# hanmekim/SceneLib2

Hardware: AMD Instinct MI355X
Metric: batched MonoSLAM frames/sec (320x240, 100 feat) (higher is better)
Workload: dtype f64

## Files before the change

scenelib2_amd/csrc/sl2_ekf_update.hip:

```cpp
#include "sl2_common.hpp"
#include "sl2_chol_diag.hpp"

namespace sl2 {

typedef double v4d __attribute__((ext_vector_type(4)));

__device__ __forceinline__ v4d mfma_f64(double a, double b, v4d c) {
  return __builtin_amdgcn_mfma_f64_16x16x4f64(a, b, c, 0, 0, 0);
}

#ifdef SL2_TESTING
#define SL2_EKF_TEST_SECTION 1
#include "sl2_ekf_update_testing.inc"
#undef SL2_EKF_TEST_SECTION
#endif

constexpr int kASBatch = 4;

template <int NQ, int BATCH>
__global__ void __launch_bounds__(1024) k_build_AS(const double* __restrict__ P, const double* __restrict__ f_Hx,
                                                  const double* __restrict__ f_Hy, const double* __restrict__ f_nu,
                                                  const double* __restrict__ f_R, const int* __restrict__ succ_idx,
                                                  const int* __restrict__ m_count, double* __restrict__ At,
                                                  double* __restrict__ St, const int* __restrict__ f_hcol,
                                                  const int* __restrict__ pos_err_any, int N, int ld, int mld) {
  extern __shared__ double sAt[];
  const int b = blockIdx.x;
  const int cnt = m_count[b];
  if (cnt == 0) return;
  const int m = 2 * cnt, mp = (m + 31) / 32 * 32;
  const int t = threadIdx.x;
  double* Ab = At + (size_t)b * mld * ld;
  double* Sb = St + (size_t)b * mld * mld;
  const double* Pb = P + (size_t)b * ld * ld;
  const int* sidx = succ_idx + (size_t)b * N;
  const int* hcol = (pos_err_any[b] != 0) ? f_hcol + (size_t)b * N : nullptr;
  double pc[NQ][7];
#pragma unroll
  for (int q = 0; q < NQ; ++q) {
    const int i = t + q * (int)blockDim.x;
#pragma unroll
    for (int c = 0; c < 7; ++c) pc[q][c] = (i >= ld) ? 0.0 : ((i < 13) ? Pb[(size_t)i * ld + c] : Pb[(size_t)c * ld + i]);
  }
  double hx[7], hy[3], Rn = 0.0;
  int posa = 0;
  if (t < m) {
    const int fa = sidx[t >> 1];
    const size_t fia = (size_t)b * N + fa;
    posa = hcol ? hcol[fa] : 13 + 3 * fa;
#pragma unroll
    for (int c = 0; c < 7; ++c) hx[c] = (hcol && (unsigned)(c - posa) < 3u) ? 0.0 : f_Hx[fia * 14 + (t & 1) * 7 + c];
#pragma unroll
    for (int c = 0; c < 3; ++c) hy[c] = f_Hy[fia * 6 + (t & 1) * 3 + c];
    Rn = f_R[fia];
  }
  const int nbatch = (cnt + BATCH - 1) / BATCH, per = (nbatch + (int)gridDim.y - 1) / (int)gridDim.y;
  const int jbeg = (int)blockIdx.y * per * BATCH;
  const int jend = (jbeg + per * BATCH < cnt) ? jbeg + per * BATCH : cnt;
  for (int j0 = jbeg; j0 < jend; j0 += BATCH) {
    const int nb = (jend - j0 < BATCH) ? jend - j0 : BATCH;
#pragma unroll
    for (int jj = 0; jj < BATCH; ++jj) {
      if (jj < nb) {
        const int f = sidx[j0 + jj];
        const size_t fi = (size_t)b * N + f;
        const int pos = hcol ? hcol[f] : 13 + 3 * f;
#pragma unroll
        for (int q = 0; q < NQ; ++q) {
          const int i = t + q * (int)blockDim.x;
          if (i < ld) {
            double py[3];
#pragma unroll
            for (int c = 0; c < 3; ++c)
              py[c] = Pb[(size_t)(pos + c) * ld + i];
#pragma unroll
            for (int r = 0; r < 2; ++r) {
              double acc = 0.0;
#pragma unroll
              for (int c = 0; c < 7; ++c) acc += pc[q][c] * ((hcol && (unsigned)(c - pos) < 3u) ? 0.0 : f_Hx[fi * 14 + r * 7 + c]);
#pragma unroll
              for (int c = 0; c < 3; ++c) acc += py[c] * f_Hy[fi * 6 + r * 3 + c];
              if (i == ld - 1) acc = f_nu[fi * 2 + r];
              Ab[(size_t)(2 * (j0 + jj) + r) * ld + i] = acc;
              sAt[(2 * jj + r) * ld + i] = acc;
            }
          }
        }
      }
    }
    __syncthreads();
    if (t < mp) {
#pragma unroll
      for (int kk = 0; kk < 2 * BATCH; ++kk) {
        const int k = 2 * j0 + kk;
        if (kk < 2 * nb && (t | 31) >= k) {
          double v = 0.0;
          if (t < m) {
            const double* arow = sAt + kk * ld;
            double acc = 0.0;
#pragma unroll
            for (int c = 0; c < 7; ++c) acc += hx[c] * arow[c];
#pragma unroll
            for (int c = 0; c < 3; ++c) acc += hy[c] * arow[posa + c];
            if (t == k) acc += Rn;
            v = acc;
          }
          Sb[(size_t)k * mld + t] = v;
        }
      }
    }
    __syncthreads();
  }
  if (blockIdx.y != 0) return;
  for (int k = m; k < mp; ++k) {
#pragma unroll
    for (int q = 0; q < NQ; ++q) {
      const int i = t + q * (int)blockDim.x;
      if (i < ld) Ab[(size_t)k * ld + i] = 0.0;
    }
    if (t < mp && (t | 31) >= k) Sb[(size_t)k * mld + t] = (t == k) ? 1.0 : 0.0;
  }
}

constexpr int kAheadEntry = 24;
constexpr int kAheadLdsMax = 40960;

template <int BATCH>
struct AheadRows { double v[BATCH][3]; };

__device__ __forceinline__ int ahead_pos(const double* en) { return *(const int*)(en + 23); }

__device__ __forceinline__ double ahead_lane(double v, int l) {
  return __hiloint2double(__builtin_amdgcn_readlane(__double2hiint(v), l), __builtin_amdgcn_readlane(__double2loint(v), l));
}

typedef __attribute__((address_space(1))) double ahead_gdouble;
__device__ __forceinline__ ahead_gdouble* ahead_at(const double* row, int t) {
  unsigned long long a = (unsigned long long)row;
  asm("" : "+s"(a));
  return (ahead_gdouble*)(a + (unsigned)t * (unsigned)sizeof(double));
}

template <int BATCH, bool FULL>
__device__ __forceinline__ void ahead_load(AheadRows<BATCH>& w, const double* __restrict__ Pb, const double* tab, int j0, int nb,
                                           int ld, int t) {
#pragma unroll
  for (int jj = 0; jj < BATCH; ++jj) {
    if (FULL || jj < nb) {
      const int pos = __builtin_amdgcn_readfirstlane(ahead_pos(tab + (j0 + jj) * kAheadEntry));
#pragma unroll
      for (int c = 0; c < 3; ++c) w.v[jj][c] = *ahead_at(Pb + (size_t)(pos + c) * ld, t);
    }
  }
}

template <int BATCH, bool FULL, bool REFILL>
__device__ __forceinline__ void ahead_rows(AheadRows<BATCH>& w, const double (&pc)[7], const double* tab, const double* __restrict__ Pb,
                                           double* __restrict__ Ab, double* sAt, int j0, int nb, int ld, int t) {
#pragma unroll
  for (int jj = 0; jj < BATCH; ++jj) {
    if (FULL || jj < nb) {
      double en = 0.0;
      if ((t & 63) < kAheadEntry) en = tab[(j0 + jj) * kAheadEntry + (t & 63)];
#pragma unroll
      for (int r = 0; r < 2; ++r) {
        double acc = 0.0;
#pragma unroll
        for (int c = 0; c < 7; ++c) acc += pc[c] * ahead_lane(en, r * 7 + c);
#pragma unroll
        for (int c = 0; c < 3; ++c) acc += w.v[jj][c] * ahead_lane(en, 14 + r * 3 + c);
        if (t == ld - 1) acc = ahead_lane(en, 20 + r);
        *ahead_at(Ab + (size_t)(2 * (j0 + jj) + r) * ld, t) = acc;
        sAt[(2 * jj + r) * ld + t] = acc;
      }
      if (REFILL && jj < BATCH - 1) {
        const int pos = __builtin_amdgcn_readfirstlane(ahead_pos(tab + (j0 + BATCH + jj) * kAheadEntry));
#pragma unroll
        for (int c = 0; c < 3; ++c) w.v[jj][c] = *ahead_at(Pb + (size_t)(pos + c) * ld, t);
      }
    }
  }
}

template <int BATCH>
__device__ __forceinline__ void ahead_refill_last(AheadRows<BATCH>& w, const double* tab, const double* __restrict__ Pb, int j0, int ld, int t) {
  const int pos = __builtin_amdgcn_readfirstlane(ahead_pos(tab + (j0 + 2 * BATCH - 1) * kAheadEntry));
#pragma unroll
  for (int c = 0; c < 3; ++c) w.v[BATCH - 1][c] = *ahead_at(Pb + (size_t)(pos + c) * ld, t);
}

template <int BATCH>
__device__ __forceinline__ void ahead_S(const double* sAt, const double* tab, double* __restrict__ Sb, int j0, int nb, int m, int mp,
                                        int ld, int mld, int t) {
  __syncthreads();
  double hx[7], hy[3], Rn = 0.0;
  int posa = 0;
  if (t < m) {
    const double* en = tab + (t >> 1) * kAheadEntry;
#pragma unroll
    for (int c = 0; c < 7; ++c) hx[c] = en[(t & 1) * 7 + c];
#pragma unroll
    for (int c = 0; c < 3; ++c) hy[c] = en[14 + (t & 1) * 3 + c];
    Rn = en[22];
    posa = ahead_pos(en);
  }
#pragma unroll
  for (int kk = 0; kk < 2 * BATCH; ++kk) {
    const int k = 2 * j0 + kk;
    if (kk < 2 * nb) {
      const double* arow = sAt + kk * ld;
      if (t < mp && (t | 31) >= k) {
        double v = 0.0;
        if (t < m) {
          double acc = 0.0;
#pragma unroll
          for (int c = 0; c < 7; ++c) acc += hx[c] * arow[c];
#pragma unroll
          for (int c = 0; c < 3; ++c) acc += hy[c] * arow[posa + c];
          if (t == k) acc += Rn;
          v = acc;
        }
        Sb[(size_t)k * mld + t] = v;
      }
    }
  }
  __syncthreads();
}

template <int BATCH>
__global__ void __launch_bounds__(1024) __attribute__((amdgpu_waves_per_eu(6, 8))) k_build_AS_ahead(const double* __restrict__ P, const double* __restrict__ f_Hx,
                                                        const double* __restrict__ f_Hy, const double* __restrict__ f_nu,
                                                        const double* __restrict__ f_R, const int* __restrict__ succ_idx,
                                                        const int* __restrict__ m_count, double* __restrict__ At,
                                                        double* __restrict__ St, const int* __restrict__ f_hcol,
                                                        const int* __restrict__ pos_err_any, int N, int ld, int mld, int tab_cap) {
  extern __shared__ double sAt[];
  const int b = blockIdx.x;
  int cnt = m_count[b];
  if (cnt == 0) return;
  cnt = cnt > tab_cap ? tab_cap : cnt;
  const int m = 2 * cnt, mp = (m + 31) / 32 * 32;
  const int t = threadIdx.x;
  double* Ab = At + (size_t)b * mld * ld;
  double* Sb = St + (size_t)b * mld * mld;
  const double* Pb = P + (size_t)b * ld * ld;
  double* tab = sAt + 2 * BATCH * ld;
  {
    const int* sidx = succ_idx + (size_t)b * N;
    const int* hcol = (pos_err_any[b] != 0) ? f_hcol + (size_t)b * N : nullptr;
    for (int idx = t; idx < cnt * kAheadEntry; idx += (int)blockDim.x) {
      const int j = idx / kAheadEntry, el = idx - j * kAheadEntry;
      const int f = sidx[j];
      const size_t fi = (size_t)b * N + f;
      const int pos = hcol ? hcol[f] : 13 + 3 * f;
      double v;
      if (el < 14) v = (hcol && (unsigned)(el % 7 - pos) < 3u) ? 0.0 : f_Hx[fi * 14 + el];
      else if (el < 20) v = f_Hy[fi * 6 + (el - 14)];
      else if (el < 22) v = f_nu[fi * 2 + (el - 20)];
      else if (el == 22) v = f_R[fi];
      else v = __longlong_as_double((long long)pos);
      tab[idx] = v;
    }
  }
  double pc[7];
#pragma unroll
  for (int c = 0; c < 7; ++c) pc[c] = (t < 13) ? Pb[(size_t)t * ld + c] : Pb[(size_t)c * ld + t];
  __syncthreads();
  const int nfull = cnt / BATCH, rem = cnt - nfull * BATCH;
  AheadRows<BATCH> w;
  if (nfull > 0) {
    ahead_load<BATCH, true>(w, Pb, tab, 0, BATCH, ld, t);
    int k = 0;
    for (; k + 1 < nfull; ++k) {
      ahead_rows<BATCH, true, true>(w, pc, tab, Pb, Ab, sAt, k * BATCH, BATCH, ld, t);
      ahead_S<BATCH>(sAt, tab, Sb, k * BATCH, BATCH, m, mp, ld, mld, t);
      ahead_refill_last<BATCH>(w, tab, Pb, k * BATCH, ld, t);
    }
    ahead_rows<BATCH, true, false>(w, pc, tab, Pb, Ab, sAt, k * BATCH, BATCH, ld, t);
    ahead_S<BATCH>(sAt, tab, Sb, k * BATCH, BATCH, m, mp, ld, mld, t);
  }
  if (rem > 0) {
    ahead_load<BATCH, false>(w, Pb, tab, nfull * BATCH, rem, ld, t);
    ahead_rows<BATCH, false, false>(w, pc, tab, Pb, Ab, sAt, nfull * BATCH, rem, ld, t);
    ahead_S<BATCH>(sAt, tab, Sb, nfull * BATCH, rem, m, mp, ld, mld, t);
  }
  for (int k = m; k < mp; ++k) {
    Ab[(size_t)k * ld + t] = 0.0;
    if (t < mp && (t | 31) >= k) Sb[(size_t)k * mld + t] = (t == k) ? 1.0 : 0.0;
  }
}


#ifdef SL2_TESTING
#define SL2_EKF_TEST_SECTION 3
#include "sl2_ekf_update_testing.inc"
#undef SL2_EKF_TEST_SECTION
#endif


__device__ __forceinline__ double fast_rcp(double p) {
  double r = __builtin_amdgcn_rcp(p);
  r = __builtin_fma(__builtin_fma(-p, r, 1.0), r, r);
  r = __builtin_fma(__builtin_fma(-p, r, 1.0), r, r);
  return r;
// ... 384 lines not shown
  const int nblk = (2 * cnt + 31) / 32;
  const int tid = threadIdx.x, lane = tid & 63, wave = tid >> 6;
  const int lo = lane & 15, hi = lane >> 4;
  const int i0 = ct * 16;
  const double* Ab = At + (size_t)b * mld * ld;
  double* Vb = Vt + (size_t)b * mld * ld;
  const double* Sb = St + (size_t)b * mld * mld;
  const double* Lb = LinvT + (size_t)b * nblk_max * 1024;
  __shared__ double sV[kKsMaxBlocks][32 * 16];
  __shared__ double sPart[4][32 * 16];
  auto load_l = [&](int J, int K, double (&a0)[8], double (&a1)[8]) {
    const double* lt = Sb + (size_t)(K * 32 + hi) * mld + J * 32 + lo;
#pragma unroll
    for (int s8 = 0; s8 < 8; ++s8) { a0[s8] = lt[(size_t)(4 * s8) * mld]; a1[s8] = lt[(size_t)(4 * s8) * mld + 16]; }
  };
  auto load_linv = [&](int J, double (&l0)[4], double (&l1)[8]) {
    const double* li = Lb + (size_t)J * 1024 + hi * 32 + lo;
#pragma unroll
    for (int s8 = 0; s8 < 8; ++s8) { if (s8 < 4) l0[s8] = li[4 * s8 * 32]; l1[s8] = li[4 * s8 * 32 + 16]; }
  };
  v4d at[2];
  double li0[4], li1[8];
  double pa0[8], pa1[8];
  int pJ = wave + 1, pK = wave;
  if (pJ < nblk) load_l(pJ, pK, pa0, pa1);
  if (wave == 0) {
#pragma unroll
    for (int jt = 0; jt < 2; ++jt)
#pragma unroll
      for (int r = 0; r < 4; ++r) at[jt][r] = Ab[(size_t)(16 * jt + hi + 4 * r) * ld + i0 + lo];
    load_linv(0, li0, li1);
  }
  for (int J = 0; J < nblk; ++J) {
    v4d acc[2];
    acc[0] = (v4d){0, 0, 0, 0};
    acc[1] = (v4d){0, 0, 0, 0};
    for (int K = wave; K < J; K += 4) {
      double a0[8], a1[8];
#pragma unroll
      for (int s8 = 0; s8 < 8; ++s8) { a0[s8] = pa0[s8]; a1[s8] = pa1[s8]; }
      if (K + 4 < J) { pJ = J; pK = K + 4; } else { pJ = J + 1; pK = wave; }
      if (pJ < nblk) load_l(pJ, pK, pa0, pa1);
      const double* vk = &sV[K][hi * 16 + lo];
#pragma unroll
      for (int s8 = 0; s8 < 8; ++s8) {
        const double bv = vk[4 * s8 * 16];
        acc[0] = mfma_f64(a0[s8], bv, acc[0]);
        acc[1] = mfma_f64(a1[s8], bv, acc[1]);
      }
    }
#pragma unroll
    for (int jt = 0; jt < 2; ++jt)
#pragma unroll
      for (int r = 0; r < 4; ++r) sPart[wave][(16 * jt + hi + 4 * r) * 16 + lo] = acc[jt][r];
    __syncthreads();
    if (wave == 0) {
      v4d rhs[2];
#pragma unroll
      for (int jt = 0; jt < 2; ++jt)
#pragma unroll
        for (int r = 0; r < 4; ++r) {
          const int e = (16 * jt + hi + 4 * r) * 16 + lo;
          rhs[jt][r] = at[jt][r] - (((sPart[0][e] + sPart[1][e]) + sPart[2][e]) + sPart[3][e]);
        }
      double l0[4], l1[8];
#pragma unroll
      for (int s8 = 0; s8 < 8; ++s8) { if (s8 < 4) l0[s8] = li0[s8]; l1[s8] = li1[s8]; }
      if (J + 1 < nblk) {
#pragma unroll
        for (int jt = 0; jt < 2; ++jt)
#pragma unroll
          for (int r = 0; r < 4; ++r) at[jt][r] = Ab[(size_t)((J + 1) * 32 + 16 * jt + hi + 4 * r) * ld + i0 + lo];
        load_linv(J + 1, li0, li1);
      }
      v4d out[2];
      out[0] = (v4d){0, 0, 0, 0};
      out[1] = (v4d){0, 0, 0, 0};
#pragma unroll
      for (int s8 = 0; s8 < 8; ++s8) {
        const double bv = rhs[s8 >> 2][s8 & 3];
        if (s8 < 4) out[0] = mfma_f64(l0[s8], bv, out[0]);
        out[1] = mfma_f64(l1[s8], bv, out[1]);
      }
#pragma unroll
      for (int jt = 0; jt < 2; ++jt)
#pragma unroll
        for (int r = 0; r < 4; ++r) {
          const int row = 16 * jt + hi + 4 * r;
          sV[J][row * 16 + lo] = out[jt][r];
          Vb[(size_t)(J * 32 + row) * ld + i0 + lo] = out[jt][r];
        }
    }
    __syncthreads();
  }
}

static int launch_fwdsub_lds(sl2_engine* e, int B, bool* done) {
  *done = true;
  if (e->nblk_max <= kKsMaxBlocks && (long long)B * (e->ld / 16) <= 160 && !e->root->no_ksplit) {
    LaunchScope ls(e, "k_fwdsub_ksplit", true);
    hipLaunchKernelGGL(k_fwdsub_ksplit, dim3(xcd_grid(e->ld / 16, B)), dim3(256), 0, e->stream, e->At, e->Vt, e->St, e->LinvT,
                       e->m_gate, e->ld, e->mld, e->nblk_max, B);
    SL2_HIP(hipGetLastError());
    return SL2_OK;
  }
  if (e->nblk_max > e->root->group_from) { *done = false; return SL2_OK; }
  const dim3 grid(xcd_grid(e->ld / 64, B)), block(256);
  LaunchScope ls(e, "k_fwdsub_lds", true);
#define SL2_FWD_CASE(NBV)                                                                                           \
  case NBV:                                                                                                         \
    hipLaunchKernelGGL((k_fwdsub_lds<NBV>), grid, block, 0, e->stream, e->At, e->Vt, e->St, e->LinvT, e->m_gate, \
                       e->ld, e->mld, e->nblk_max, B, 0, 0, e->ld / 64, NBV);                                       \
    break;
  switch (e->nblk_max) {
    SL2_FWD_CASE(1) SL2_FWD_CASE(2) SL2_FWD_CASE(3) SL2_FWD_CASE(4) SL2_FWD_CASE(5) SL2_FWD_CASE(6) SL2_FWD_CASE(7)
    SL2_FWD_CASE(8) SL2_FWD_CASE(9) SL2_FWD_CASE(10) SL2_FWD_CASE(11) SL2_FWD_CASE(12) SL2_FWD_CASE(13)
    default: break;
  }
#undef SL2_FWD_CASE
  SL2_HIP(hipGetLastError());
  return SL2_OK;
}

constexpr int kSyrkKC = 16;

__device__ __forceinline__ void kpanel_product(const double* __restrict__ A, size_t lda, const double* __restrict__ Bm, size_t ldb,
                                               int nchunk, bool idle, int wi, int wj, double (&sAB)[2][2][kSyrkKC * 64],
                                               v4d (&acc)[2][2]) {
  const int tid = threadIdx.x, lane = tid & 63;
  const int lo = lane & 15, hi = lane >> 4;
  const int kr = tid >> 4, c2 = (tid & 15) * 2;
  const double* gA = A + (size_t)kr * lda + c2;
  const double* gB = Bm + (size_t)kr * ldb + c2;
  struct Stage { double2 a0, a1, b0, b1; };
  auto stage_load = [&](int chunk) {
    Stage r;
    r.a0 = *(const double2*)(gA + (size_t)chunk * kSyrkKC * lda); r.a1 = *(const double2*)(gA + (size_t)chunk * kSyrkKC * lda + 32);
    r.b0 = *(const double2*)(gB + (size_t)chunk * kSyrkKC * ldb); r.b1 = *(const double2*)(gB + (size_t)chunk * kSyrkKC * ldb + 32);
    return r;
  };
  auto stage_store = [&](int buf, const Stage& r) {
    const int cs = c2 ^ ((kr & 1) << 4);
    *(double2*)&sAB[buf][0][kr * 64 + cs] = r.a0;
    *(double2*)&sAB[buf][0][kr * 64 + 32 + cs] = r.a1;
    *(double2*)&sAB[buf][1][kr * 64 + cs] = r.b0;
    *(double2*)&sAB[buf][1][kr * 64 + 32 + cs] = r.b1;
  };
  auto chunk_mfma = [&](int buf) {
    const int sw = (hi & 1) << 4;
    const double* pa = &sAB[buf][0][hi * 64 + wi + lo];
    const double* pb = &sAB[buf][1][hi * 64 + wj + lo];
#pragma unroll
    for (int ks = 0; ks < kSyrkKC / 4; ++ks) {
      const double a0 = pa[ks * 256 + sw], a1 = pa[ks * 256 + (sw ^ 16)];
      const double b0 = pb[ks * 256 + sw], b1 = pb[ks * 256 + (sw ^ 16)];
      acc[0][0] = mfma_f64(a0, b0, acc[0][0]);
      acc[0][1] = mfma_f64(a0, b1, acc[0][1]);
      acc[1][0] = mfma_f64(a1, b0, acc[1][0]);
      acc[1][1] = mfma_f64(a1, b1, acc[1][1]);
    }
  };
  if (nchunk <= 0) return;
  Stage r0 = stage_load(0);
  Stage r1 = r0;
  if (nchunk > 1) r1 = stage_load(1);
  for (int ch = 0; ch < nchunk; ch += 2) {
    stage_store(0, r0);
    __syncthreads();
    if (ch + 2 < nchunk) r0 = stage_load(ch + 2);
    if (!idle) chunk_mfma(0);
    if (ch + 1 >= nchunk) break;
    stage_store(1, r1);
    __syncthreads();
    if (ch + 3 < nchunk) r1 = stage_load(ch + 3);
    if (!idle) chunk_mfma(1);
  }
}

__global__ void __launch_bounds__(256, 4) k_fwd_gemm(double* __restrict__ At, const double* __restrict__ Vt,
                                                  const double* __restrict__ St, const int* __restrict__ m_count, int ld, int mld,
                                                  int B, int J0, int nrt) {
  int b, t;
  const int ntc = ld / 64;
  if (!xcd_map(nrt * ntc, B, &b, &t)) return;
  const int cnt = m_count[b];
  if (cnt == 0) return;
  const int mp = (2 * cnt + 31) / 32 * 32;
  const int R0 = J0 * 32;
  const int r0 = R0 + (t / ntc) * 64, c0 = (t % ntc) * 64;
  if (r0 >= mp) return;
  const int tid = threadIdx.x, lane = tid & 63, wave = tid >> 6;
  const int lo = lane & 15, hi = lane >> 4;
  const int wi = (wave >> 1) * 32, wj = (wave & 1) * 32;
  double* Ab = At + (size_t)b * mld * ld;
  const double* Vb = Vt + (size_t)b * mld * ld;
  const double* Sb = St + (size_t)b * mld * mld;
  __shared__ double sAB[2][2][kSyrkKC * 64];
  v4d acc[2][2];
  for (int it = 0; it < 2; ++it) for (int jt = 0; jt < 2; ++jt) acc[it][jt] = (v4d){0, 0, 0, 0};
  kpanel_product(Sb + r0, (size_t)mld, Vb + c0, (size_t)ld, R0 / kSyrkKC, false, wi, wj, sAB, acc);
#pragma unroll
  for (int it = 0; it < 2; ++it)
#pragma unroll
    for (int jt = 0; jt < 2; ++jt)
#pragma unroll
      for (int r = 0; r < 4; ++r) {
        double* q = Ab + (size_t)(r0 + wi + 16 * it + hi + 4 * r) * ld + c0 + wj + 16 * jt + lo;
        *q -= acc[it][jt][r];
      }
}

__global__ void __launch_bounds__(256) k_chol_syrk(double* __restrict__ St, const int* __restrict__ m_count, int mld, int B,
                                                   int k0, int kp, int c0) {
  int b, t;
  const int nt = (mld - c0) / 64;
  if (!xcd_map(nt * (nt + 1) / 2, B, &b, &t)) return;
  const int cnt = m_count[b];
  if (cnt == 0) return;
  const int mp = (2 * cnt + 31) / 32 * 32;
  int ti = 0;
  while (t > ti) { t -= ti + 1; ++ti; }
  const int tj = t;
  const int j0 = c0 + tj * 64, i0 = c0 + ti * 64;
  if (j0 >= mp || i0 >= mp) return;
  const int tid = threadIdx.x, lane = tid & 63, wave = tid >> 6;
  const int lo = lane & 15, hi = lane >> 4;
  const int wj = (wave >> 1) * 32, wi = (wave & 1) * 32;
  double* Sb = St + (size_t)b * mld * mld;
  __shared__ double sAB[2][2][kSyrkKC * 64];
  v4d acc[2][2];
  for (int a = 0; a < 2; ++a) for (int c = 0; c < 2; ++c) acc[a][c] = (v4d){0, 0, 0, 0};
  const int kvalid = (mp - k0 < kp) ? mp - k0 : kp;
  const bool idle = (ti == tj) && (wj > wi);
  kpanel_product(Sb + (size_t)k0 * mld + j0, (size_t)mld, Sb + (size_t)k0 * mld + i0, (size_t)mld, kvalid / kSyrkKC, idle, wj, wi, sAB,
                 acc);
  if (idle) return;
#pragma unroll
  for (int a = 0; a < 2; ++a)
#pragma unroll
    for (int c = 0; c < 2; ++c)
#pragma unroll
      for (int r = 0; r < 4; ++r) {
        double* q = Sb + (size_t)(j0 + wj + 16 * a + hi + 4 * r) * mld + i0 + wi + 16 * c + lo;
        *q -= acc[a][c][r];
      }
}

constexpr int kCholPanelBlocks = 4;

static int launch_chol_panels(sl2_engine* e, int B) {
  const int pb = e->root->chol_panel == 8 ? 8 : kCholPanelBlocks;
  for (int p0 = 0; p0 < e->nblk_max; p0 += pb) {
    const int nb = e->nblk_max - p0 < pb ? e->nblk_max - p0 : pb;
    {
      LaunchScope ls(e, "k_chol_left", true);
      hipLaunchKernelGGL(k_chol_left, dim3(B), dim3(256), 0, e->stream, e->St, e->LinvT, e->m_gate, e->mld, e->nblk_max, p0, nb,
                         (long long*)nullptr);
      SL2_HIP(hipGetLastError());
    }
    const int c0 = (p0 + nb) * 32;
    if (c0 >= e->mld) break;
    const int ntile = (e->mld - c0) / 64;
    {
      LaunchScope ls(e, "k_fwdsub_lds@chol", true);
      if (pb == 8)
        hipLaunchKernelGGL((k_fwdsub_lds<8>), dim3(xcd_grid(ntile, B)), dim3(256), 0, e->stream, e->St, e->St, e->St,
                           e->LinvT, e->m_gate, e->mld, e->mld, e->nblk_max, B, p0, c0, ntile, nb);
      else
        hipLaunchKernelGGL((k_fwdsub_lds<kCholPanelBlocks>), dim3(xcd_grid(ntile, B)), dim3(256), 0, e->stream, e->St, e->St, e->St,
                           e->LinvT, e->m_gate, e->mld, e->mld, e->nblk_max, B, p0, c0, ntile, nb);
      SL2_HIP(hipGetLastError());
    }
    {
      LaunchScope ls(e, "k_chol_syrk", true);
      hipLaunchKernelGGL(k_chol_syrk, dim3(xcd_grid(ntile * (ntile + 1) / 2, B)), dim3(256), 0, e->stream, e->St, e->m_gate, e->mld,
                         B, p0 * 32, nb * 32, c0);
      SL2_HIP(hipGetLastError());
    }
  }
  return SL2_OK;
}

static int launch_fwdsub_grouped(sl2_engine* e, int B) {
  const int g = e->root->fwd_group == 4 ? 4 : 8;
  for (int J0 = 0; J0 < e->nblk_max; J0 += g) {
    if (J0 > 0) {
      LaunchScope ls(e, "k_fwd_gemm", true);
      hipLaunchKernelGGL(k_fwd_gemm, dim3(xcd_grid((g / 2) * (e->ld / 64), B)), dim3(256), 0, e->stream, e->At, e->Vt, e->St,
                         e->m_gate, e->ld, e->mld, B, J0, g / 2);
      SL2_HIP(hipGetLastError());
    }
    LaunchScope ls(e, "k_fwdsub_lds", true);
    if (g == 4)
      hipLaunchKernelGGL((k_fwdsub_lds<4>), dim3(xcd_grid(e->ld / 64, B)), dim3(256), 0, e->stream, e->At, e->Vt, e->St, e->LinvT,
                         e->m_gate, e->ld, e->mld, e->nblk_max, B, J0, 0, e->ld / 64, 4);
    else
      hipLaunchKernelGGL((k_fwdsub_lds<8>), dim3(xcd_grid(e->ld / 64, B)), dim3(256), 0, e->stream, e->At, e->Vt, e->St, e->LinvT,
                         e->m_gate, e->ld, e->mld, e->nblk_max, B, J0, 0, e->ld / 64, 8);
    SL2_HIP(hipGetLastError());
  }
  return SL2_OK;
}


__global__ void __launch_bounds__(256, 4) k_syrk(const double* __restrict__ Vt, double* __restrict__ P, double* __restrict__ x,
                                              const int* __restrict__ m_count, int ld, int mld, int B,
                                              const int* __restrict__ n_slots, int ppos
#ifdef SL2_CHOL_TRACE
                                              , long long* trace
#endif
                                              ) {
#ifdef SL2_CHOL_TRACE
  struct Stamp {
    long long* p;
    __device__ Stamp(long long* q) : p(q) { if (p && threadIdx.x == 0) p[2 * blockIdx.x] = (long long)__builtin_readcyclecounter(); }
    __device__ ~Stamp() { if (p && threadIdx.x == 0) p[2 * blockIdx.x + 1] = (long long)__builtin_readcyclecounter(); }
  } stamp(trace);
#endif
  int b, t;
  const int ntl = ld / 64;
  if (!xcd_map(ntl * (ntl + 1) / 2, B, &b, &t)) return;
  const int cnt = m_count[b];
  if (cnt == 0) return;
  const int mp = (2 * cnt + kSyrkKC - 1) / kSyrkKC * kSyrkKC;
  const int nks_last = (2 * cnt - (mp - kSyrkKC) + 3) >> 2;
  int tj = 0;
  while (t > tj) { t -= tj + 1; ++tj; }
  const int ti = t;
  const int n_live = 13 + 3 * n_slots[b];
  {
    const int t_lo = (n_live + 63) >> 6, t_hi = ppos >> 6;
    if ((ti >= t_lo && ti < t_hi) || (tj >= t_lo && tj < t_hi)) return;
  }
  const int tid = threadIdx.x;
  const int lane = tid & 63, wave = tid >> 6;
  const int lo = lane & 15, hi = lane >> 4;
  const int wi = (wave >> 1) * 32, wj = (wave & 1) * 32;
  const double* Vb = Vt + (size_t)b * mld * ld;
  double* Pb = P + (size_t)b * ld * ld;
  __shared__ double sAB[2][2][kSyrkKC * 64];
  const int kr = tid >> 4, c2 = (tid & 15) * 2;
  const double* gA = Vb + (size_t)kr * ld + ti * 64 + c2;
  const double* gB = Vb + (size_t)kr * ld + tj * 64 + c2;
  struct Stage { double2 a0, a1, b0, b1; };
  auto stage_load = [&](int chunk) {
    Stage r;
    const size_t off = (size_t)chunk * kSyrkKC * ld;
    r.a0 = *(const double2*)(gA + off); r.a1 = *(const double2*)(gA + off + 32);
    r.b0 = *(const double2*)(gB + off); r.b1 = *(const double2*)(gB + off + 32);
    return r;
  };
  auto stage_store = [&](int buf, const Stage& r) {
    const int cs = c2 ^ ((kr & 1) << 4);
    *(double2*)&sAB[buf][0][kr * 64 + cs] = r.a0;
    *(double2*)&sAB[buf][0][kr * 64 + 32 + cs] = r.a1;
    *(double2*)&sAB[buf][1][kr * 64 + cs] = r.b0;
    *(double2*)&sAB[buf][1][kr * 64 + 32 + cs] = r.b1;
  };
  Stage r0 = stage_load(0);
  const int i0 = ti * 64 + wi, j0 = tj * 64 + wj;
  const int b_lo = (n_live + 31) >> 5, b_hi = ppos >> 5;
  const bool idle = ((ti == tj) && (wi > wj)) || ((i0 >> 5) >= b_lo && (i0 >> 5) < b_hi) || ((j0 >> 5) >= b_lo && (j0 >> 5) < b_hi);
  v4d acc[2][2];
  for (int it = 0; it < 2; ++it) for (int jt = 0; jt < 2; ++jt) acc[it][jt] = (v4d){0, 0, 0, 0};
  const int nchunk = mp / kSyrkKC;
  Stage r1 = r0;
  if (nchunk > 1) r1 = stage_load(1);
  const bool interior = (i0 + 32 < ld && j0 + 32 < ld);
  const bool diagw = (ti == tj) && (wi == wj) && interior;
  auto chunk_mfma = [&](int buf, int nks) {
    const int sw = (hi & 1) << 4;
    const double* pa = &sAB[buf][0][hi * 64 + wi + lo];
    const double* pb = &sAB[buf][1][hi * 64 + wj + lo];
#pragma unroll
    for (int ks = 0; ks < kSyrkKC / 4; ++ks) {
      if (ks < nks) {
        const double a0 = pa[ks * 256 + sw], a1 = pa[ks * 256 + (sw ^ 16)];
        const double b0 = pb[ks * 256 + sw], b1 = pb[ks * 256 + (sw ^ 16)];
        acc[0][0] = mfma_f64(a0, b0, acc[0][0]);
        acc[0][1] = mfma_f64(a0, b1, acc[0][1]);
        if (!diagw) acc[1][0] = mfma_f64(a1, b0, acc[1][0]);
        acc[1][1] = mfma_f64(a1, b1, acc[1][1]);
      }
    }
  };
  double pold[2][2][4];
  auto fetch_tile = [&]() {
    const double* prow = Pb + (size_t)(i0 + hi) * ld + j0 + lo;
#pragma unroll
    for (int it = 0; it < 2; ++it)
#pragma unroll
      for (int jt = 0; jt < 2; ++jt)
#pragma unroll
        for (int r = 0; r < 4; ++r) pold[it][jt][r] = prow[(size_t)(16 * it + 4 * r) * ld + 16 * jt];
  };
  const bool want_tile = !idle;
  for (int ch = 0; ch < nchunk; ch += 2) {
    stage_store(0, r0);
    __syncthreads();
    if (ch + 2 < nchunk) r0 = stage_load(ch + 2);
    if (!idle) chunk_mfma(0, (ch + 1 >= nchunk) ? nks_last : kSyrkKC / 4);
    if (ch + 1 >= nchunk) break;
    stage_store(1, r1);
    __syncthreads();
    if (ch + 3 < nchunk) r1 = stage_load(ch + 3);
    if (!idle) chunk_mfma(1, (ch + 2 >= nchunk) ? nks_last : kSyrkKC / 4);
  }
  const int lastbuf = (nchunk - 1) & 1;
  if (want_tile) fetch_tile();
  if (idle) return;
  const bool mirror = (ti != tj) || (wi != wj);
  auto plain = [&](int it, int jt) { return interior || ((i0 + 16 * it + 16 < ld) && (j0 + 16 * jt + 16 < ld)); };
  {
    double* prow = Pb + (size_t)(i0 + hi) * ld + j0 + lo;
#pragma unroll
    for (int it = 0; it < 2; ++it)
#pragma unroll
      for (int jt = 0; jt < 2; ++jt) {
        if (!plain(it, jt)) continue;
#pragma unroll
        for (int r = 0; r < 4; ++r) {
          if (diagw && it == 1 && jt == 0) continue;
          const double pn = pold[it][jt][r] - acc[it][jt][r];
          prow[(size_t)(16 * it + 4 * r) * ld + 16 * jt] = pn;
          acc[it][jt][r] = pn;
        }
      }
    if (mirror || diagw) {
      const int other = lastbuf ^ 1;
      double* sM = &sAB[other][0][0] + wave * (16 * 17);
      double* pm = Pb + (size_t)(j0 + hi) * ld + i0 + lo;
#pragma unroll
      for (int it = 0; it < 2; ++it)
#pragma unroll
        for (int jt = 0; jt < 2; ++jt) {
          if (diagw && !(it == 0 && jt == 1)) continue;
          if (!plain(it, jt)) continue;
#pragma unroll
          for (int r = 0; r < 4; ++r) sM[lo * 17 + 4 * r + hi] = acc[it][jt][r];
          asm volatile("s_waitcnt lgkmcnt(0)" ::: "memory");
#pragma unroll
          for (int k = 0; k < 4; ++k) pm[(size_t)(16 * jt + 4 * k) * ld + 16 * it] = sM[(4 * k + hi) * 17 + lo];
          asm volatile("s_waitcnt lgkmcnt(0)" ::: "memory");
        }
    }
    if (interior) return;
  }
  double* xb = x + (size_t)b * ld;
#pragma unroll
  for (int it = 0; it < 2; ++it)
#pragma unroll
    for (int jt = 0; jt < 2; ++jt) {
      if (plain(it, jt)) continue;
#pragma unroll
      for (int r = 0; r < 4; ++r) {
        const int row = i0 + 16 * it + hi + 4 * r, col = j0 + 16 * jt + lo;
        const double v = acc[it][jt][r];
        if (col == ld - 1) {
          if (row != ld - 1) xb[row] += v;
        } else if (row != ld - 1) {
          const double pn = pold[it][jt][r] - v;
          Pb[(size_t)row * ld + col] = pn;
          if (mirror) Pb[(size_t)col * ld + row] = pn;
        }
      }
    }
}

#ifdef SL2_TESTING
#define SL2_EKF_TEST_SECTION 9
#include "sl2_ekf_update_testing.inc"
#undef SL2_EKF_TEST_SECTION
#endif


static int launch_update_range(sl2_engine* e) {
  const int B = e->B;
#ifdef SL2_TESTING
  const int build_variant = e->root->build_variant, chol_variant = e->root->chol_variant, fwd_variant = e->root->fwd_variant;
#else
  const int chol_variant = 1, fwd_variant = 1;
#endif
#ifdef SL2_TESTING
  if (build_variant == 0) {
    {
      LaunchScope ls(e, "k_build_A", true);
      const int threads = e->ld <= 512 ? e->ld : 512;
      hipLaunchKernelGGL(k_build_A, dim3(B), dim3(threads), 0, e->stream, e->P, e->f_Hx, e->f_Hy, e->f_nu, e->succ_idx,
                         e->m_gate, e->At, e->N, e->ld, e->mld);
      SL2_HIP(hipGetLastError());
    }
    {
      LaunchScope ls(e, "k_build_S");
      dim3 grid(e->mld / 32, (e->mld + 255) / 256, B);
      hipLaunchKernelGGL(k_build_S, grid, dim3(256), 0, e->stream, e->At, e->f_Hx, e->f_Hy, e->f_R, e->succ_idx, e->m_gate,
                         e->St, e->N, e->ld, e->mld);
      SL2_HIP(hipGetLastError());
    }
  } else
#endif
  {
    LaunchScope ls(e, "k_build_AS", true);
    int nsplit = B >= 1024 ? 1 : (3072 + B - 1) / B;
    if (e->root->build_split > 0) nsplit = e->root->build_split;
    if (nsplit < 1) nsplit = 1;
    const int nbatch_max = (e->N + kASBatch - 1) / kASBatch;
    if (nsplit > nbatch_max) nsplit = nbatch_max;
    int ahead = 0;
    if (nsplit == 1 && e->ld <= 1024 && e->root->build_ahead != 0) {
      const size_t tab = sizeof(double) * kAheadEntry * e->nsel_max;
      if (sizeof(double) * 2 * 4 * e->ld + tab <= (size_t)kAheadLdsMax) ahead = 4;
      else if (sizeof(double) * 2 * 2 * e->ld + tab <= (size_t)kAheadLdsMax) ahead = 2;
    }
    if (ahead) {
      size_t shm = sizeof(double) * (2 * ahead * e->ld + kAheadEntry * e->nsel_max);
      if ((size_t)e->root->build_lds_min > shm) shm = (size_t)e->root->build_lds_min;
      if (ahead == 4)
        hipLaunchKernelGGL((k_build_AS_ahead<4>), dim3(B), dim3(e->ld), shm, e->stream, e->P, e->f_Hx, e->f_Hy, e->f_nu, e->f_R,
                           e->succ_idx, e->m_gate, e->At, e->St, e->f_hcol, e->pos_err_any, e->N, e->ld, e->mld, e->nsel_max);
      else
        hipLaunchKernelGGL((k_build_AS_ahead<2>), dim3(B), dim3(e->ld), shm, e->stream, e->P, e->f_Hx, e->f_Hy, e->f_nu, e->f_R,
                           e->succ_idx, e->m_gate, e->At, e->St, e->f_hcol, e->pos_err_any, e->N, e->ld, e->mld, e->nsel_max);
    } else if (e->ld <= 1024) {
      size_t shm = sizeof(double) * 2 * kASBatch * e->ld;
      if ((size_t)e->root->build_lds_min > shm) shm = (size_t)e->root->build_lds_min;
      hipLaunchKernelGGL((k_build_AS<1, kASBatch>), dim3(B, nsplit), dim3(e->ld), shm, e->stream, e->P, e->f_Hx, e->f_Hy, e->f_nu, e->f_R,
                         e->succ_idx, e->m_gate, e->At, e->St, e->f_hcol, e->pos_err_any, e->N, e->ld, e->mld);
    } else {
      const size_t shm = sizeof(double) * 2 * 2 * e->ld;
      hipLaunchKernelGGL((k_build_AS<2, 2>), dim3(B, nsplit), dim3(1024), shm, e->stream, e->P, e->f_Hx, e->f_Hy, e->f_nu, e->f_R,
                         e->succ_idx, e->m_gate, e->At, e->St, e->f_hcol, e->pos_err_any, e->N, e->ld, e->mld);
    }
    SL2_HIP(hipGetLastError());
  }
  if (e->nblk_max > e->root->panel_from && chol_variant >= 1 && e->mld % 64 == 0 && e->nblk_max % kCholPanelBlocks == 0) {
    int rc = launch_chol_panels(e, B);
    if (rc != SL2_OK) return rc;
  } else if (e->nblk_max <= e->root->panel_from && chol_variant == 1) {
    LaunchScope ls(e, "k_chol_left", true);
    hipLaunchKernelGGL(k_chol_left, dim3(B), dim3(256), 0, e->stream, e->St, e->LinvT, e->m_gate, e->mld, e->nblk_max, 0,
                       e->nblk_max, (long long*)e->root->chol_trace);
    SL2_HIP(hipGetLastError());
  } else {
#ifdef SL2_TESTING
    {
      for (int J = 0; J < e->nblk_max; ++J) {
        {
          LaunchScope ls(e, "k_chol_diag");
          hipLaunchKernelGGL(k_chol_diag, dim3(B), dim3(64), 0, e->stream, e->St, e->LinvT, e->m_gate, e->mld, e->nblk_max, J);
          SL2_HIP(hipGetLastError());
        }
        const int rem = e->nblk_max - 1 - J;
        if (rem > 0) {
          {
            LaunchScope ls(e, "k_chol_panel");
            hipLaunchKernelGGL(k_chol_panel, dim3(rem, B), dim3(64), 0, e->stream, e->St, e->LinvT, e->m_gate, e->mld,
                               e->nblk_max, J);
            SL2_HIP(hipGetLastError());
          }
          {
            LaunchScope ls(e, "k_chol_trail");
            hipLaunchKernelGGL(k_chol_trail, dim3(rem * (rem + 1) / 2, B), dim3(64), 0, e->stream, e->St, e->m_gate, e->mld, J);
            SL2_HIP(hipGetLastError());
          }
        }
      }
    }
#else
    set_error("launch_update: no factorisation for this system size (sl2_create should have padded it)");
    return SL2_ERR_INVALID;
#endif
  }
  {
    bool done = false;
    if (fwd_variant == 1) {
      int rc = launch_fwdsub_lds(e, B, &done);
      if (rc != SL2_OK) return rc;
      if (!done && e->mld % 64 == 0) {
        rc = launch_fwdsub_grouped(e, B);
        if (rc != SL2_OK) return rc;
        done = true;
      }
    }
    if (!done) {
#ifdef SL2_TESTING
      LaunchScope ls(e, "k_fwdsub", true);
      hipLaunchKernelGGL(k_fwdsub, dim3(xcd_grid(e->ld / 64, B)), dim3(128), 0, e->stream, e->At, e->Vt, e->St, e->LinvT,
                         e->m_gate, e->ld, e->mld, e->nblk_max, B);
      SL2_HIP(hipGetLastError());
#else
      set_error("launch_update: no substitution kernel for this system size (sl2_create should have padded it)");
      return SL2_ERR_INVALID;
#endif
    }
  }
  {
    LaunchScope ls(e, "k_syrk", true);
    const int nt = e->ld / 64;
#ifdef SL2_CHOL_TRACE
    static const bool trace_syrk = getenv("SL2_TRACE_SYRK") != nullptr;
    hipLaunchKernelGGL(k_syrk, dim3(xcd_grid(nt * (nt + 1) / 2, B)), dim3(256), 0, e->stream, e->Vt, e->P, e->x, e->m_gate,
                       e->ld, e->mld, B, e->n_slots, e->ppos, trace_syrk ? (long long*)e->root->chol_trace : nullptr);
#else
    hipLaunchKernelGGL(k_syrk, dim3(xcd_grid(nt * (nt + 1) / 2, B)), dim3(256), 0, e->stream, e->Vt, e->P, e->x, e->m_gate,
                       e->ld, e->mld, B, e->n_slots, e->ppos);
#endif
    SL2_HIP(hipGetLastError());
  }
  return SL2_OK;
}

int launch_update(sl2_engine* e) { return launch_update_range(e); }

int launch_syrk_on(sl2_engine* e, const double* Vt, double* P) {
  const int nt = e->ld / 64;
#ifdef SL2_CHOL_TRACE
  hipLaunchKernelGGL(k_syrk, dim3(xcd_grid(nt * (nt + 1) / 2, e->B)), dim3(256), 0, e->stream, Vt, P, e->x, e->m_count, e->ld, e->mld, e->B,
                     e->n_slots, e->ppos, (long long*)nullptr);
#else
  hipLaunchKernelGGL(k_syrk, dim3(xcd_grid(nt * (nt + 1) / 2, e->B)), dim3(256), 0, e->stream, Vt, P, e->x, e->m_count, e->ld, e->mld, e->B,
                     e->n_slots, e->ppos);
#endif
  SL2_HIP(hipGetLastError());
  return SL2_OK;
}

}

#ifdef SL2_TESTING
#define SL2_EKF_TEST_SECTION 10
#include "sl2_ekf_update_testing.inc"
#undef SL2_EKF_TEST_SECTION
#endif
```

Baseline: 1.029 million.

## Specialize SYRK k-loop for idle/diagonal waves and share A/B on diagonal tiles

Restructures the SYRK kernel's k-loop into a template-specialized lambda with compile-time idle and diagonal-wave variants. On diagonal tiles it loads and stores only the A panel to LDS and reuses it as B, which halves global and LDS traffic there. It also prefetches half of the old P tile before the last chunk's MFMAs to overlap latency, and switches addressing to 32-bit unsigned byte offsets with a wave-uniform readfirstlane. The cost is more code paths and therefore more instruction-cache pressure and register pressure.

```diff
diff --git a/scenelib2_amd/csrc/sl2_ekf_update.hip b/scenelib2_amd/csrc/sl2_ekf_update.hip
--- a/scenelib2_amd/csrc/sl2_ekf_update.hip
+++ b/scenelib2_amd/csrc/sl2_ekf_update.hip
@@ -1,5 +1,6 @@
 #include "sl2_common.hpp"
 #include "sl2_chol_diag.hpp"
+#include <type_traits>
 
 namespace sl2 {
 
@@ -990,6 +991,7 @@
   return SL2_OK;
 }
 
+typedef double v2d __attribute__((ext_vector_type(2)));
 
 __global__ void __launch_bounds__(256, 4) k_syrk(const double* __restrict__ Vt, double* __restrict__ P, double* __restrict__ x,
                                               const int* __restrict__ m_count, int ld, int mld, int B,
@@ -1021,86 +1023,108 @@
     if ((ti >= t_lo && ti < t_hi) || (tj >= t_lo && tj < t_hi)) return;
   }
   const int tid = threadIdx.x;
-  const int lane = tid & 63, wave = tid >> 6;
+  const int lane = tid & 63, wave = __builtin_amdgcn_readfirstlane(tid >> 6);
   const int lo = lane & 15, hi = lane >> 4;
   const int wi = (wave >> 1) * 32, wj = (wave & 1) * 32;
   const double* Vb = Vt + (size_t)b * mld * ld;
   double* Pb = P + (size_t)b * ld * ld;
+  const bool dtile = (ti == tj);
   __shared__ double sAB[2][2][kSyrkKC * 64];
   const int kr = tid >> 4, c2 = (tid & 15) * 2;
-  const double* gA = Vb + (size_t)kr * ld + ti * 64 + c2;
-  const double* gB = Vb + (size_t)kr * ld + tj * 64 + c2;
-  struct Stage { double2 a0, a1, b0, b1; };
-  auto stage_load = [&](int chunk) {
-    Stage r;
-    const size_t off = (size_t)chunk * kSyrkKC * ld;
-    r.a0 = *(const double2*)(gA + off); r.a1 = *(const double2*)(gA + off + 32);
-    r.b0 = *(const double2*)(gB + off); r.b1 = *(const double2*)(gB + off + 32);
-    return r;
+  const unsigned ldb = (unsigned)ld * 8u;
+  const unsigned goff = (unsigned)kr * ldb + (unsigned)c2 * 8u;
+  const char* gA = (const char*)(Vb + ti * 64);
+  const char* gB = (const char*)(Vb + tj * 64);
+  struct Stage { v2d a0, a1, b0, b1; };
+  auto stage_load = [&](Stage& r, int chunk) {
+    const size_t off = (size_t)((unsigned)chunk * kSyrkKC * ldb);
+    r.a0 = *(const v2d*)(gA + off + goff); r.a1 = *(const v2d*)(gA + off + 256 + goff);
+    if (!dtile) { r.b0 = *(const v2d*)(gB + off + goff); r.b1 = *(const v2d*)(gB + off + 256 + goff); }
   };
   auto stage_store = [&](int buf, const Stage& r) {
     const int cs = c2 ^ ((kr & 1) << 4);
-    *(double2*)&sAB[buf][0][kr * 64 + cs] = r.a0;
-    *(double2*)&sAB[buf][0][kr * 64 + 32 + cs] = r.a1;
-    *(double2*)&sAB[buf][1][kr * 64 + cs] = r.b0;
-    *(double2*)&sAB[buf][1][kr * 64 + 32 + cs] = r.b1;
+    *(v2d*)&sAB[buf][0][kr * 64 + cs] = r.a0;
+    *(v2d*)&sAB[buf][0][kr * 64 + 32 + cs] = r.a1;
+    if (!dtile) {
+      *(v2d*)&sAB[buf][1][kr * 64 + cs] = r.b0;
+      *(v2d*)&sAB[buf][1][kr * 64 + 32 + cs] = r.b1;
+    }
   };
-  Stage r0 = stage_load(0);
   const int i0 = ti * 64 + wi, j0 = tj * 64 + wj;
   const int b_lo = (n_live + 31) >> 5, b_hi = ppos >> 5;
   const bool idle = ((ti == tj) && (wi > wj)) || ((i0 >> 5) >= b_lo && (i0 >> 5) < b_hi) || ((j0 >> 5) >= b_lo && (j0 >> 5) < b_hi);
   v4d acc[2][2];
   for (int it = 0; it < 2; ++it) for (int jt = 0; jt < 2; ++jt) acc[it][jt] = (v4d){0, 0, 0, 0};
   const int nchunk = mp / kSyrkKC;
-  Stage r1 = r0;
-  if (nchunk > 1) r1 = stage_load(1);
   const bool interior = (i0 + 32 < ld && j0 + 32 < ld);
   const bool diagw = (ti == tj) && (wi == wj) && interior;
-  auto chunk_mfma = [&](int buf, int nks) {
+  const unsigned voff = (unsigned)hi * ldb + (unsigned)lo * 8u;
+  char* tile = (char*)(Pb + (size_t)i0 * ld + j0);
+  char* mtile = (char*)(Pb + (size_t)j0 * ld + i0);
+  auto quarter = [&](char* base, int rows, int cols, unsigned vo) {
+    return (double*)(base + (size_t)((unsigned)rows * ldb + (unsigned)cols * 8u) + vo);
+  };
+  auto here = [](unsigned v) { asm volatile("" : "+v"(v)); return v; };
+  double pold[2][2][4];
+  auto fetch_tile = [&](int it) {
+    const unsigned vo = here(voff);
+#pragma unroll
+    for (int jt = 0; jt < 2; ++jt)
+#pragma unroll
+      for (int r = 0; r < 4; ++r) pold[it][jt][r] = *quarter(tile, 16 * it + 4 * r, 16 * jt, vo);
+  };
+  auto chunk_mfma = [&](int buf, bool half, auto diag_tag) {
+    constexpr bool DIAGW = decltype(diag_tag)::value;
     const int sw = (hi & 1) << 4;
     const double* pa = &sAB[buf][0][hi * 64 + wi + lo];
-    const double* pb = &sAB[buf][1][hi * 64 + wj + lo];
+    const double* pb = &sAB[buf][dtile ? 0 : 1][hi * 64 + wj + lo];
 #pragma unroll
     for (int ks = 0; ks < kSyrkKC / 4; ++ks) {
-      if (ks < nks) {
-        const double a0 = pa[ks * 256 + sw], a1 = pa[ks * 256 + (sw ^ 16)];
-        const double b0 = pb[ks * 256 + sw], b1 = pb[ks * 256 + (sw ^ 16)];
-        acc[0][0] = mfma_f64(a0, b0, acc[0][0]);
-        acc[0][1] = mfma_f64(a0, b1, acc[0][1]);
-        if (!diagw) acc[1][0] = mfma_f64(a1, b0, acc[1][0]);
-        acc[1][1] = mfma_f64(a1, b1, acc[1][1]);
-      }
+      if (ks == 2 && half) break;
+      const double a0 = pa[ks * 256 + sw], a1 = pa[ks * 256 + (sw ^ 16)];
+      const double b0 = pb[ks * 256 + sw], b1 = pb[ks * 256 + (sw ^ 16)];
+      acc[0][0] = mfma_f64(a0, b0, acc[0][0]);
+      acc[0][1] = mfma_f64(a0, b1, acc[0][1]);
+      if (!DIAGW) acc[1][0] = mfma_f64(a1, b0, acc[1][0]);
+      acc[1][1] = mfma_f64(a1, b1, acc[1][1]);
     }
   };
-  double pold[2][2][4];
-  auto fetch_tile = [&]() {
-    const double* prow = Pb + (size_t)(i0 + hi) * ld + j0 + lo;
-#pragma unroll
-    for (int it = 0; it < 2; ++it)
-#pragma unroll
-      for (int jt = 0; jt < 2; ++jt)
-#pragma unroll
-        for (int r = 0; r < 4; ++r) pold[it][jt][r] = prow[(size_t)(16 * it + 4 * r) * ld + 16 * jt];
+  auto kloop = [&](auto idle_tag, auto diag_tag) {
+    constexpr bool IDLE = decltype(idle_tag)::value;
+    Stage r0, r1;
+    r0.b0 = r0.b1 = r1.b0 = r1.b1 = (v2d){0.0, 0.0};
+    stage_load(r0, 0);
+    r1.a0 = r0.a0; r1.a1 = r0.a1;
+    if (nchunk > 1) stage_load(r1, 1);
+    for (int ch = 0; ch < nchunk; ch += 2) {
+      stage_store(0, r0);
+      __syncthreads();
+      if (ch + 2 < nchunk) stage_load(r0, ch + 2);
+      if (!IDLE) {
+        const bool last = (ch + 1 >= nchunk);
+        if (last) fetch_tile(0);
+        chunk_mfma(0, last && nks_last <= 2, diag_tag);
+      }
+      if (ch + 1 >= nchunk) break;
+      stage_store(1, r1);
+      __syncthreads();
+      if (ch + 3 < nchunk) stage_load(r1, ch + 3);
+      if (!IDLE) {
+        const bool last = (ch + 2 >= nchunk);
+        if (last) fetch_tile(0);
+        chunk_mfma(1, last && nks_last <= 2, diag_tag);
+      }
+    }
   };
-  const bool want_tile = !idle;
-  for (int ch = 0; ch < nchunk; ch += 2) {
-    stage_store(0, r0);
-    __syncthreads();
-    if (ch + 2 < nchunk) r0 = stage_load(ch + 2);
-    if (!idle) chunk_mfma(0, (ch + 1 >= nchunk) ? nks_last : kSyrkKC / 4);
-    if (ch + 1 >= nchunk) break;
-    stage_store(1, r1);
-    __syncthreads();
-    if (ch + 3 < nchunk) r1 = stage_load(ch + 3);
-    if (!idle) chunk_mfma(1, (ch + 2 >= nchunk) ? nks_last : kSyrkKC / 4);
-  }
+  if (idle) { kloop(std::true_type{}, std::false_type{}); return; }
+  if (diagw) kloop(std::false_type{}, std::true_type{});
+  else kloop(std::false_type{}, std::false_type{});
   const int lastbuf = (nchunk - 1) & 1;
-  if (want_tile) fetch_tile();
-  if (idle) return;
+  fetch_tile(1);
   const bool mirror = (ti != tj) || (wi != wj);
+  const unsigned vo = here(voff);
   auto plain = [&](int it, int jt) { return interior || ((i0 + 16 * it + 16 < ld) && (j0 + 16 * jt + 16 < ld)); };
   {
-    double* prow = Pb + (size_t)(i0 + hi) * ld + j0 + lo;
 #pragma unroll
     for (int it = 0; it < 2; ++it)
 #pragma unroll
@@ -1110,14 +1134,13 @@
         for (int r = 0; r < 4; ++r) {
           if (diagw && it == 1 && jt == 0) continue;
           const double pn = pold[it][jt][r] - acc[it][jt][r];
-          prow[(size_t)(16 * it + 4 * r) * ld + 16 * jt] = pn;
+          *quarter(tile, 16 * it + 4 * r, 16 * jt, vo) = pn;
           acc[it][jt][r] = pn;
         }
       }
     if (mirror || diagw) {
       const int other = lastbuf ^ 1;
       double* sM = &sAB[other][0][0] + wave * (16 * 17);
-      double* pm = Pb + (size_t)(j0 + hi) * ld + i0 + lo;
 #pragma unroll
       for (int it = 0; it < 2; ++it)
 #pragma unroll
@@ -1128,13 +1151,14 @@
           for (int r = 0; r < 4; ++r) sM[lo * 17 + 4 * r + hi] = acc[it][jt][r];
           asm volatile("s_waitcnt lgkmcnt(0)" ::: "memory");
 #pragma unroll
-          for (int k = 0; k < 4; ++k) pm[(size_t)(16 * jt + 4 * k) * ld + 16 * it] = sM[(4 * k + hi) * 17 + lo];
+          for (int k = 0; k < 4; ++k) *quarter(mtile, 16 * jt + 4 * k, 16 * it, vo) = sM[(4 * k + hi) * 17 + lo];
           asm volatile("s_waitcnt lgkmcnt(0)" ::: "memory");
         }
     }
     if (interior) return;
   }
   double* xb = x + (size_t)b * ld;
+  const unsigned voffT = here((unsigned)lo * ldb + (unsigned)hi * 8u);
 #pragma unroll
   for (int it = 0; it < 2; ++it)
 #pragma unroll
@@ -1148,8 +1172,8 @@
           if (row != ld - 1) xb[row] += v;
         } else if (row != ld - 1) {
           const double pn = pold[it][jt][r] - v;
-          Pb[(size_t)row * ld + col] = pn;
-          if (mirror) Pb[(size_t)col * ld + row] = pn;
+          *quarter(tile, 16 * it + 4 * r, 16 * jt, vo) = pn;
+          if (mirror) *(double*)(mtile + (size_t)((unsigned)(16 * jt) * ldb + (unsigned)(16 * it + 4 * r) * 8u) + voffT) = pn;
         }
       }
     }
```

After: 1.032 million (median of 3 runs). No clear change (+0.3%).
